# RaphaelHaddad/Real-Time-Brain-Inspired-Video-Memory

Hardware: AMD Instinct MI355X
Metric: frame-embeddings/sec (+ kNN queries/sec, see knn) (higher is better)
Workload: dtype f16; 1 GPU; BASELINE configs[1]: ViT-B/16-224 encoder fp16, chunks of 16 frames, cosine top-10 over a 100000-row x 768 fp16 memory shard per GPU; chunk_size=16, memory_rows_per_gpu=100000, top_k=10, parallelism=single GPU

## Files before the change

include/vidmem.h:

```cpp
#ifndef VIDMEM_H
#define VIDMEM_H

#include <stddef.h>
#include <stdint.h>

#ifdef __cplusplus
extern "C" {
#endif

typedef struct vm_ctx vm_ctx;
typedef struct vm_encoder vm_encoder;
typedef struct vm_memory vm_memory;

enum vm_status {
    VM_OK = 0,
    VM_ERR_INVALID = -1,
    VM_ERR_HIP = -2,
    VM_ERR_NOMEM = -3,
    VM_ERR_UNSUPPORTED = -4,
    VM_ERR_NO_DEVICE = -5
};
enum vm_dtype { VM_F16 = 0, VM_BF16 = 1, VM_F32 = 2  };
enum vm_act { VM_ACT_GELU = 0, VM_ACT_QUICK_GELU = 1 };
enum vm_layout { VM_LAYOUT_CHW = 0, VM_LAYOUT_PATCHES = 1 };
enum vm_score_mode { VM_SCORE_RAW = 0, VM_SCORE_UNIT_INTERVAL = 1 };
enum vm_topk_flag { VM_FLAG_CERTIFIED = 0, VM_FLAG_GAP = 1, VM_FLAG_OVERFLOW = 3 };

int vm_init(int device, vm_ctx **out);
void vm_destroy(vm_ctx *ctx);
const char *vm_last_error(vm_ctx *ctx);
int vm_abi_version(void);

int vm_preprocess(vm_ctx *ctx, const uint8_t *frames_hwc_bgr, int B, int H, int W, const float mean_host[3],
                  const float std_host[3], int out_S, int dtype, int layout, int patch, int k_pad, void *out,
                  void *stream);

typedef struct vm_encoder_desc {
    int image;
    int patch;
    int hidden;
    int layers;
    int heads;
    int mlp;
    int act;
    int pre_ln;
    int patch_bias;
    int proj_dim;
    int dtype;
    float ln_eps;
} vm_encoder_desc;

int vm_encoder_create(vm_ctx *ctx, const vm_encoder_desc *desc, const void *const *weights_host, int n_weights,
                      vm_encoder **out);
void vm_encoder_destroy(vm_encoder *enc);
enum vm_encoder_option { VM_ENC_OPT_SCHEDULE = 0, VM_ENC_OPT_MICRO_BATCH = 1, VM_ENC_OPT_LAST_LAYER = 2 };
enum vm_encoder_schedule { VM_SCHED_AUTO = 0, VM_SCHED_ONE_STREAM = 1, VM_SCHED_TWO_STREAMS = 2 };
int vm_encoder_set_option(vm_encoder *enc, int option, int value);
int vm_encoder_get_option(const vm_encoder *enc, int option);
int vm_encoder_tokens(const vm_encoder *enc);
int vm_encoder_patch_k(const vm_encoder *enc);
int vm_encoder_out_dim(const vm_encoder *enc);
size_t vm_encode_workspace_bytes(const vm_encoder *enc, int B);
int vm_encode_micro_batch(const vm_encoder *enc, int B);
int vm_encode(vm_encoder *enc, const void *patches, int B, void *out_emb, int l2_normalise, void *workspace,
              size_t workspace_bytes, void *stream);

typedef struct vm_text_encoder vm_text_encoder;
typedef struct vm_text_encoder_desc {
    int vocab;
    int context;
    int hidden;
    int layers;
    int heads;
    int mlp;
    int act;
    int proj_dim;
    int eot_id;
    int dtype;
    float ln_eps;
} vm_text_encoder_desc;
int vm_text_encoder_create(vm_ctx *ctx, const vm_text_encoder_desc *desc, const void *const *weights_host,
                           int n_weights, vm_text_encoder **out);
void vm_text_encoder_destroy(vm_text_encoder *enc);
int vm_text_encoder_out_dim(const vm_text_encoder *enc);
size_t vm_text_encode_workspace_bytes(const vm_text_encoder *enc, int B, int T);
int vm_text_encode(vm_text_encoder *enc, const int32_t *token_ids, int B, int T, void *out_emb, int l2_normalise,
                   int32_t *out_flags, void *workspace, size_t workspace_bytes, void *stream);

// ... 85 lines not shown
```

real-time-brain-inspired-video-memory_amd/_lib.py:

```python
from __future__ import annotations

import ctypes as C
import os
from typing import Optional

_HERE = os.path.dirname(os.path.abspath(__file__))
LIB_PATH = os.path.join(_HERE, "libvidmem.so")
DEV_LIB_PATH = os.path.join(_HERE, "libvidmem_dev.so")

VM_OK = 0
VM_ERR_INVALID, VM_ERR_HIP, VM_ERR_NOMEM, VM_ERR_UNSUPPORTED, VM_ERR_NO_DEVICE = -1, -2, -3, -4, -5
VM_F16, VM_BF16, VM_F32 = 0, 1, 2
VM_ACT_GELU, VM_ACT_QUICK_GELU = 0, 1
VM_LAYOUT_CHW, VM_LAYOUT_PATCHES = 0, 1
VM_SCORE_RAW, VM_SCORE_UNIT_INTERVAL = 0, 1
VM_FLAG_CERTIFIED, VM_FLAG_GAP, VM_FLAG_OVERFLOW = 0, 1, 3
VM_ENC_OPT_SCHEDULE, VM_ENC_OPT_MICRO_BATCH, VM_ENC_OPT_LAST_LAYER = 0, 1, 2
VM_SCHED_AUTO, VM_SCHED_ONE_STREAM, VM_SCHED_TWO_STREAMS = 0, 1, 2
SCHEDULES = {"auto": VM_SCHED_AUTO, "one_stream": VM_SCHED_ONE_STREAM, "two_streams": VM_SCHED_TWO_STREAMS}
DTYPES = {"f16": VM_F16, "bf16": VM_BF16}

SYMBOLS = [
    "vm_init", "vm_destroy", "vm_last_error", "vm_abi_version", "vm_preprocess",
    "vm_encoder_create", "vm_encoder_destroy", "vm_encoder_set_option", "vm_encoder_get_option",
    "vm_encoder_tokens", "vm_encoder_patch_k", "vm_encoder_out_dim",
    "vm_encode_workspace_bytes", "vm_encode_micro_batch", "vm_encode",
    "vm_memory_create", "vm_memory_destroy", "vm_memory_append", "vm_memory_size", "vm_memory_capacity",
    "vm_memory_dim", "vm_memory_reset", "vm_memory_sync", "vm_memory_rows",
    "vm_memory_create_grouped", "vm_memory_append_grouped", "vm_memory_group_keys",
    "vm_topk_grouped_workspace_bytes", "vm_topk_cosine_grouped", "vm_topk_cosine_grouped_exact",
    "vm_memory_create_tagged", "vm_memory_append_tagged", "vm_memory_tags",
    "vm_novelty_workspace_bytes", "vm_memory_append_novel",
    "vm_topk_scoped_workspace_bytes", "vm_topk_cosine_scoped", "vm_topk_cosine_scoped_exact",
    "vm_topk_workspace_bytes", "vm_topk_cosine", "vm_topk_redo_workspace_bytes", "vm_topk_redo_flagged",
    "vm_topk_exact_workspace_bytes", "vm_topk_cosine_exact",
    "vm_cosine_exact", "vm_topk_select", "vm_topk_merge", "vm_profile_enable", "vm_profile_read", "vm_profile_mask", "vm_probe_mfma",
    "vm_text_encoder_create", "vm_text_encoder_destroy", "vm_text_encoder_out_dim", "vm_text_encode_workspace_bytes",
    "vm_text_encode",
]
PROF_CATS = ["preprocess", "gemm_patch", "gemm_qkv", "gemm_act", "gemm_resid", "attention", "layernorm", "pool",
             "append", "topk_scan", "topk_finalize", "topk_exact", "topk_merge", "gemm_cls"]


class VidmemError(RuntimeError):
    def __init__(self, code: int, message: str):
        super().__init__(f"libvidmem error {code}: {message}")
        self.code = code


class EncoderDesc(C.Structure):
# ... 149 lines not shown
```

real-time-brain-inspired-video-memory_amd/csrc/encoder.hip:

```cpp
#include "vm_internal.h"
#include "vm_kernels.h"

#include <type_traits>

namespace {

__device__ __forceinline__ float wave_sum(float v) {
    auto dpp_add = [](float x, auto ctrl, auto row_mask) {
        const int y = __builtin_amdgcn_update_dpp(0, __builtin_bit_cast(int, x), decltype(ctrl)::value,
                                                  decltype(row_mask)::value, 0xf, false);
        return x + __builtin_bit_cast(float, y);
    };
    using std::integral_constant;
    v = dpp_add(v, integral_constant<int, 0xB1>{}, integral_constant<int, 0xf>{});
    v = dpp_add(v, integral_constant<int, 0x4E>{}, integral_constant<int, 0xf>{});
    v = dpp_add(v, integral_constant<int, 0x141>{}, integral_constant<int, 0xf>{});
    v = dpp_add(v, integral_constant<int, 0x140>{}, integral_constant<int, 0xf>{});
    v = dpp_add(v, integral_constant<int, 0x142>{}, integral_constant<int, 0xa>{});
    v = dpp_add(v, integral_constant<int, 0x143>{}, integral_constant<int, 0xc>{});
    return __builtin_bit_cast(float, __builtin_amdgcn_readlane(__builtin_bit_cast(int, v), 63));
}

typedef float f32x4_v __attribute__((ext_vector_type(4)));
typedef unsigned u32x2_v __attribute__((ext_vector_type(2)));
// ... 90 lines not shown
                v[r][i].w += e[r][i].w;
            }
        }
        if (write_x > 1 ? row % write_x == 0 : write_x) {
            float4 *xr = reinterpret_cast<float4 *>(x32 + (size_t)row * rstride * H);
#pragma unroll
            for (int i = 0; i < VPL; ++i) st_f4<NT>(xr + lane + 64 * i, v[r][i]);
        }
        float sum = 0.f;
#pragma unroll
        for (int i = 0; i < VPL; ++i) sum += (v[r][i].x + v[r][i].y) + (v[r][i].z + v[r][i].w);
        const float mean = wave_sum(sum) / (float)H;
        float sq = 0.f;
#pragma unroll
        for (int i = 0; i < VPL; ++i) {
            const float a = v[r][i].x - mean, b = v[r][i].y - mean, c = v[r][i].z - mean, e = v[r][i].w - mean;
            sq += (a * a + b * b) + (c * c + e * e);
        }
        const float rstd = rsqrtf(wave_sum(sq) / (float)H + eps);
#pragma unroll
        for (int i = 0; i < VPL; ++i) {
            uint16_t o[4] = {E::from_float((v[r][i].x - mean) * rstd * g4[i].x + b4[i].x),
                             E::from_float((v[r][i].y - mean) * rstd * g4[i].y + b4[i].y),
                             E::from_float((v[r][i].z - mean) * rstd * g4[i].z + b4[i].z),
                             E::from_float((v[r][i].w - mean) * rstd * g4[i].w + b4[i].w)};
            uint2 pk;
            __builtin_memcpy(&pk, o, 8);
            st_u2<NT>(reinterpret_cast<uint2 *>(out16 + (size_t)row * rstride * H) + lane + 64 * i, pk);
        }
    }
}

template <int DT, int VPL, bool NT>
__global__ void __launch_bounds__(256, 8) resid_layernorm_lowreg_kernel(float *__restrict__ x32,
                                                                        const uint16_t *__restrict__ delta16,
                                                                        const uint16_t *__restrict__ deltaB16,
                                                                        int write_x, const float *__restrict__ gamma,
                                                                        const float *__restrict__ beta, float eps,
                                                                        uint16_t *__restrict__ out16, int rows, int H,
                                                                        int rstride) {
    using E = vm_elem<DT>;
    const int lane = threadIdx.x & 63;
    const int row = blockIdx.x * 4 + (threadIdx.x >> 6);
    if (row >= rows) return;
    const size_t base = (size_t)row * rstride * H;
    float4 v[VPL];
    const float4 *xr = reinterpret_cast<const float4 *>(x32 + base);
#pragma unroll
    for (int i = 0; i < VPL; ++i) v[i] = ld_f4<NT>(xr + lane + 64 * i);
    if (delta16) {
        float4 d[VPL];
#pragma unroll
        for (int i = 0; i < VPL; ++i) d[i] = load4_16<VM_F16, NT>(delta16 + base + 4 * (lane + 64 * i));
#pragma unroll
        for (int i = 0; i < VPL; ++i) {
            v[i].x += d[i].x;
            v[i].y += d[i].y;
            v[i].z += d[i].z;
            v[i].w += d[i].w;
        }
    }
    if (deltaB16) {
        float4 d[VPL];
#pragma unroll
        for (int i = 0; i < VPL; ++i) d[i] = load4_16<VM_F16, NT>(deltaB16 + base + 4 * (lane + 64 * i));
#pragma unroll
        for (int i = 0; i < VPL; ++i) {
            v[i].x += d[i].x;
            v[i].y += d[i].y;
            v[i].z += d[i].z;
            v[i].w += d[i].w;
        }
    }
    if (write_x > 1 ? row % write_x == 0 : write_x) {
        float4 *xw = reinterpret_cast<float4 *>(x32 + base);
#pragma unroll
        for (int i = 0; i < VPL; ++i) st_f4<NT>(xw + lane + 64 * i, v[i]);
    }
    float sum = 0.f;
#pragma unroll
    for (int i = 0; i < VPL; ++i) sum += (v[i].x + v[i].y) + (v[i].z + v[i].w);
    const float mean = wave_sum(sum) / (float)H;
    float sq = 0.f;
#pragma unroll
    for (int i = 0; i < VPL; ++i) {
        const float a = v[i].x - mean, b = v[i].y - mean, c = v[i].z - mean, e = v[i].w - mean;
        sq += (a * a + b * b) + (c * c + e * e);
    }
    const float rstd = rsqrtf(wave_sum(sq) / (float)H + eps);
#pragma unroll
    for (int i = 0; i < VPL; ++i) {
        const float4 g4 = reinterpret_cast<const float4 *>(gamma)[lane + 64 * i];
        const float4 b4 = reinterpret_cast<const float4 *>(beta)[lane + 64 * i];
        uint16_t o[4] = {E::from_float((v[i].x - mean) * rstd * g4.x + b4.x),
                         E::from_float((v[i].y - mean) * rstd * g4.y + b4.y),
                         E::from_float((v[i].z - mean) * rstd * g4.z + b4.z),
                         E::from_float((v[i].w - mean) * rstd * g4.w + b4.w)};
        uint2 pk;
        __builtin_memcpy(&pk, o, 8);
        st_u2<NT>(reinterpret_cast<uint2 *>(out16 + base) + lane + 64 * i, pk);
    }
}

template <int DT, int VPL>
__global__ void __launch_bounds__(256) embed_kernel(const uint16_t *__restrict__ patch16, const float *__restrict__ cls,
                                                    const float *__restrict__ pos, const float *__restrict__ pre_g,
                                                    const float *__restrict__ pre_b, float eps, int pre_ln,
                                                    float *__restrict__ x32, int rows, int T, int H) {
    const int lane = threadIdx.x & 63;
    const int row = blockIdx.x * 4 + (threadIdx.x >> 6);
    if (row >= rows) return;
    const int frame = row / T, tok = row - frame * T;
    float4 v[VPL];
#pragma unroll
    for (int i = 0; i < VPL; ++i) {
        const int c = lane + 64 * i;
        const float4 p4 = reinterpret_cast<const float4 *>(pos + (size_t)tok * H)[c];
        float4 e4;
        if (tok == 0)
            e4 = reinterpret_cast<const float4 *>(cls)[c];
        else
            e4 = load4_16<VM_F16>(patch16 + ((size_t)frame * (T - 1) + tok - 1) * H + 4 * c);
        v[i] = make_float4(e4.x + p4.x, e4.y + p4.y, e4.z + p4.z, e4.w + p4.w);
    }
    if (pre_ln) {
        float sum = 0.f;
#pragma unroll
        for (int i = 0; i < VPL; ++i) sum += (v[i].x + v[i].y) + (v[i].z + v[i].w);
        const float mean = wave_sum(sum) / (float)H;
        float sq = 0.f;
#pragma unroll
        for (int i = 0; i < VPL; ++i) {
            const float a = v[i].x - mean, b = v[i].y - mean, c = v[i].z - mean, d = v[i].w - mean;
            sq += (a * a + b * b) + (c * c + d * d);
// ... 101 lines not shown
        const int tt = t0 + lane;
        const int v = tt < T ? ids[(size_t)b * T + tt] : 0;
        const unsigned long long hit = __ballot(tt < T && v == eot_id);
        if (hit && first == T) first = t0 + __ffsll((long long)hit) - 1;
        clamped |= __any(tt < T && (v < 0 || v >= vocab)) != 0;
    }
    if (lane == 0) {
        pool_row[b] = first < T ? first : 0;
        if (flags) flags[b] = (clamped ? 1 : 0) | (first < T ? 0 : 2);
    }
}

}

#define VM_VPL_SWITCH(H, CALL)                                                                     \
    switch ((H) / 256) {                                                                           \
        case 1: CALL(1); break;                                                                    \
        case 2: CALL(2); break;                                                                    \
        case 3: CALL(3); break;                                                                    \
        case 4: CALL(4); break;                                                                    \
        default: return vm_fail(ctx, VM_ERR_UNSUPPORTED, "row width %d (need 256..1024, %%256)", H); \
    }

int vm_resid_layernorm(vm_ctx *ctx, int dtype, float *x32, const uint16_t *delta16, const uint16_t *deltaB16,
                       int write_x, const float *gamma, const float *beta, float eps, uint16_t *out16, int rows, int H,
                       hipStream_t st, int rstride, int lowreg) {
    constexpr int RPW = 2;
    const int blocks = (rows + 4 * RPW - 1) / (4 * RPW);
    if (H % 256 != 0) return vm_fail(ctx, VM_ERR_UNSUPPORTED, "row width %d", H);
    vm_prof_scope prof(ctx, VM_PROF_LAYERNORM, st);
    static const int lowreg_env = (int)VM_DEV_ENV("LN_LOWREG", 1);
    if (lowreg != 0 && lowreg_env != 0) {
        const int blk = (rows + 3) / 4;
#define RLNL(V)                                                                                                          \
    if (dtype == VM_F16)                                                                                                 \
        resid_layernorm_lowreg_kernel<VM_F16, V, true><<<blk, 256, 0, st>>>(x32, delta16, deltaB16, write_x, gamma, beta, eps, out16, rows, H, rstride); \
    else                                                                                                                 \
        resid_layernorm_lowreg_kernel<VM_BF16, V, true><<<blk, 256, 0, st>>>(x32, delta16, deltaB16, write_x, gamma, beta, eps, out16, rows, H, rstride)
        VM_VPL_SWITCH(H, RLNL)
#undef RLNL
        VM_LAUNCH_CHECK(ctx);
        return VM_OK;
    }
    static const int nt_env = (int)VM_DEV_ENV("LN_NT", 1);
    const bool nt = nt_env && (size_t)rows * H * 4 > ((size_t)64 << 20);
#define RLN16(V) resid_layernorm_kernel<VM_F16, V, RPW, false><<<blocks, 256, 0, st>>>(x32, delta16, deltaB16, write_x, gamma, beta, eps, out16, rows, H, rstride)
#define RLNB16(V) resid_layernorm_kernel<VM_BF16, V, RPW, false><<<blocks, 256, 0, st>>>(x32, delta16, deltaB16, write_x, gamma, beta, eps, out16, rows, H, rstride)
#define RLN16N(V) resid_layernorm_kernel<VM_F16, V, RPW, true><<<blocks, 256, 0, st>>>(x32, delta16, deltaB16, write_x, gamma, beta, eps, out16, rows, H, rstride)
#define RLNB16N(V) resid_layernorm_kernel<VM_BF16, V, RPW, true><<<blocks, 256, 0, st>>>(x32, delta16, deltaB16, write_x, gamma, beta, eps, out16, rows, H, rstride)
    if (dtype == VM_F16) {
        if (nt) { VM_VPL_SWITCH(H, RLN16N) } else { VM_VPL_SWITCH(H, RLN16) }
    } else {
        if (nt) { VM_VPL_SWITCH(H, RLNB16N) } else { VM_VPL_SWITCH(H, RLNB16) }
    }
#undef RLN16
#undef RLNB16
#undef RLN16N
#undef RLNB16N
    VM_LAUNCH_CHECK(ctx);
    return VM_OK;
}

int vm_embed(vm_ctx *ctx, int dtype, const uint16_t *patch16, const float *cls, const float *pos, const float *pre_g,
             const float *pre_b, float eps, int pre_ln, float *x32, int B, int T, int H, hipStream_t st) {
    const int rows = B * T, blocks = (rows + 3) / 4;
    if (H % 256 != 0) return vm_fail(ctx, VM_ERR_UNSUPPORTED, "row width %d", H);
// ... 35 lines not shown
    const int rows = B * T, blocks = (rows + 3) / 4;
    if (H % 256 != 0) return vm_fail(ctx, VM_ERR_UNSUPPORTED, "row width %d", H);
    vm_prof_scope prof(ctx, VM_PROF_LAYERNORM, st);
#define TEMB(V) text_embed_kernel<V><<<blocks, 256, 0, st>>>(ids, tok, pos, vocab, eot_id, x32, pool_row, flags, rows, T, H)
    VM_VPL_SWITCH(H, TEMB)
#undef TEMB
    VM_LAUNCH_CHECK(ctx);
    return VM_OK;
}

struct LayerW {
    float *ln1_g, *ln1_b, *qkv_b, *proj_b, *ln2_g, *ln2_b, *fc1_b, *fc2_b;
    uint16_t *qkv_w, *proj_w, *fc1_w, *fc2_w;
};
static void layer_sizes(size_t H, size_t M, size_t lsz[12]) {
    const size_t v[12] = {H * 4, H * 4, 3 * H * H * 2, 3 * H * 4, H * H * 2, H * 4,
                          H * 4, H * 4, M * H * 2,     M * 4,     H * M * 2, H * 4};
    for (int i = 0; i < 12; ++i) lsz[i] = v[i];
}
static void bind_layer(LayerW &w, char *b, const size_t o[12]) {
    w.ln1_g = (float *)(b + o[0]);
    w.ln1_b = (float *)(b + o[1]);
    w.qkv_w = (uint16_t *)(b + o[2]);
    w.qkv_b = (float *)(b + o[3]);
    w.proj_w = (uint16_t *)(b + o[4]);
    w.proj_b = (float *)(b + o[5]);
    w.ln2_g = (float *)(b + o[6]);
    w.ln2_b = (float *)(b + o[7]);
    w.fc1_w = (uint16_t *)(b + o[8]);
    w.fc1_b = (float *)(b + o[9]);
    w.fc2_w = (uint16_t *)(b + o[10]);
    w.fc2_b = (float *)(b + o[11]);
}
struct vm_encoder {
    vm_ctx *ctx;
    vm_encoder_desc d;
    int tokens, patches, patch_k, out_dim;
    char *blob;
    uint16_t *patch_w, *proj_w;
    float *patch_b, *cls, *pos, *pre_g, *pre_b, *ln_g, *ln_b;
    LayerW *layers;
    int micro_batch;
    int cls_last;
    int schedule;
    hipStream_t side[2];
    hipEvent_t ev_fork, ev_join[2], ev_phase;
};

static int round_up(int x, int a) { return (x + a - 1) / a * a; }

extern "C" int vm_encoder_create(vm_ctx *ctx, const vm_encoder_desc *desc, const void *const *wp, int n_weights,
                                 vm_encoder **out) {
    if (!ctx || !desc || !wp || !out) return VM_ERR_INVALID;
    const vm_encoder_desc &d = *desc;
    if (d.hidden % 256 != 0 || d.hidden > 1024 || d.heads * 64 != d.hidden)
        return vm_fail(ctx, VM_ERR_UNSUPPORTED, "hidden=%d heads=%d: need hidden %% 256 == 0, <= 1024, head dim 64",
                       d.hidden, d.heads);
    if (d.mlp % 128 != 0 || d.image % d.patch != 0 || d.layers <= 0 || d.image % 8 != 0)
        return vm_fail(ctx, VM_ERR_UNSUPPORTED, "bad mlp/image/patch/layers");
    if (d.dtype != VM_F16 && d.dtype != VM_BF16) return vm_fail(ctx, VM_ERR_INVALID, "bad dtype");
    if (d.proj_dim < 0 || d.proj_dim % 8 != 0) return vm_fail(ctx, VM_ERR_UNSUPPORTED, "proj_dim %d", d.proj_dim);
    if (n_weights != 9 + 12 * d.layers)
        return vm_fail(ctx, VM_ERR_INVALID, "expected %d weight pointers, got %d", 9 + 12 * d.layers, n_weights);
    VM_HIP(ctx, hipSetDevice(ctx->device));
    vm_encoder *e = new vm_encoder();
    memset(e, 0, sizeof(*e));
    e->ctx = ctx;
    e->d = d;
    const int g = d.image / d.patch;
    e->patches = g * g;
    e->tokens = e->patches + 1;
    e->patch_k = round_up(3 * d.patch * d.patch, 64);
    e->out_dim = d.proj_dim ? d.proj_dim : d.hidden;
    if (e->tokens > 592) {
        const int tokens = e->tokens;
        delete e;
        return vm_fail(ctx, VM_ERR_UNSUPPORTED, "%d tokens per frame > 592", tokens);
    }
    e->micro_batch = 0;
    e->cls_last = 3;
    e->schedule = VM_SCHED_AUTO;
    {
        hipError_t he = hipSuccess;
        for (int i = 0; i < 2 && he == hipSuccess; ++i) {
            he = hipStreamCreateWithFlags(&e->side[i], hipStreamNonBlocking);
            if (he == hipSuccess) he = hipEventCreateWithFlags(&e->ev_join[i], hipEventDisableTiming);
        }
        if (he == hipSuccess) he = hipEventCreateWithFlags(&e->ev_fork, hipEventDisableTiming);
        if (he == hipSuccess) he = hipEventCreateWithFlags(&e->ev_phase, hipEventDisableTiming);
        if (he != hipSuccess) {
            vm_encoder_destroy(e);
            return vm_fail(ctx, VM_ERR_HIP, "encoder streams: %s", hipGetErrorString(he));
        }
    }
    const size_t H = d.hidden, M = d.mlp;
    auto a256 = [](size_t b) { return vm_align_up(b, 256); };
    size_t total = 0;
    auto take = [&](size_t bytes) {
        size_t off = total;
        total += a256(bytes);
        return off;
    };
    const size_t o_patch_w = take(H * e->patch_k * 2), o_patch_b = take(H * 4), o_cls = take(H * 4),
                 o_pos = take((size_t)e->tokens * H * 4), o_pre_g = take(H * 4), o_pre_b = take(H * 4),
                 o_ln_g = take(H * 4), o_ln_b = take(H * 4), o_proj = take((size_t)(d.proj_dim ? d.proj_dim : 0) * H * 2);
    struct LO {
        size_t o[12];
    };
    LO *lo = new LO[d.layers];
    size_t lsz[12];
    layer_sizes(H, M, lsz);
    for (int l = 0; l < d.layers; ++l)
        for (int i = 0; i < 12; ++i) lo[l].o[i] = take(lsz[i]);
    hipError_t er = hipMalloc((void **)&e->blob, total);
    if (er != hipSuccess) {
        delete[] lo;
        delete e;
        return vm_fail(ctx, VM_ERR_NOMEM, "encoder weights: hipMalloc(%zu) failed", total);
    }
    auto copy = [&](size_t off, const void *src, size_t bytes) -> hipError_t {
        if (bytes == 0) return hipSuccess;
        if (!src) return hipErrorInvalidValue;
// ... 5 lines not shown
    if (er == hipSuccess) er = copy(o_pos, wp[3], (size_t)e->tokens * H * 4);
    if (er == hipSuccess && d.pre_ln) er = copy(o_pre_g, wp[4], H * 4);
    if (er == hipSuccess && d.pre_ln) er = copy(o_pre_b, wp[5], H * 4);
    if (er == hipSuccess) er = copy(o_ln_g, wp[6], H * 4);
    if (er == hipSuccess) er = copy(o_ln_b, wp[7], H * 4);
    if (er == hipSuccess && d.proj_dim) er = copy(o_proj, wp[8], (size_t)d.proj_dim * H * 2);
    e->layers = new LayerW[d.layers];
    for (int l = 0; l < d.layers && er == hipSuccess; ++l) {
        for (int i = 0; i < 12 && er == hipSuccess; ++i) er = copy(lo[l].o[i], wp[9 + 12 * l + i], lsz[i]);
        bind_layer(e->layers[l], e->blob, lo[l].o);
    }
    delete[] lo;
    if (er != hipSuccess) {
        vm_encoder_destroy(e);
        return vm_fail(ctx, VM_ERR_HIP, "encoder weight copy failed: %s (null or short weight pointer?)",
                       hipGetErrorString(er));
    }
    char *b = e->blob;
    e->patch_w = (uint16_t *)(b + o_patch_w);
    e->patch_b = (float *)(b + o_patch_b);
    e->cls = (float *)(b + o_cls);
    e->pos = (float *)(b + o_pos);
    e->pre_g = (float *)(b + o_pre_g);
    e->pre_b = (float *)(b + o_pre_b);
    e->ln_g = (float *)(b + o_ln_g);
    e->ln_b = (float *)(b + o_ln_b);
    e->proj_w = d.proj_dim ? (uint16_t *)(b + o_proj) : nullptr;
    *out = e;
    return VM_OK;
}

extern "C" void vm_encoder_destroy(vm_encoder *e) {
    if (!e) return;
    for (int i = 0; i < 2; ++i) {
        if (e->side[i]) (void)hipStreamDestroy(e->side[i]);
        if (e->ev_join[i]) (void)hipEventDestroy(e->ev_join[i]);
    }
    if (e->ev_fork) (void)hipEventDestroy(e->ev_fork);
    if (e->ev_phase) (void)hipEventDestroy(e->ev_phase);
    if (e->blob) (void)hipFree(e->blob);
    delete[] e->layers;
    delete e;
}

extern "C" int vm_encoder_set_option(vm_encoder *e, int option, int value) {
    if (!e) return VM_ERR_INVALID;
    switch (option) {
        case VM_ENC_OPT_SCHEDULE:
            if (value != VM_SCHED_AUTO && value != VM_SCHED_ONE_STREAM && value != VM_SCHED_TWO_STREAMS)
                return vm_fail(e->ctx, VM_ERR_INVALID, "VM_ENC_OPT_SCHEDULE: %d", value);
            e->schedule = value;
            return VM_OK;
        case VM_ENC_OPT_MICRO_BATCH:
            if (value < 0) return vm_fail(e->ctx, VM_ERR_INVALID, "VM_ENC_OPT_MICRO_BATCH: %d", value);
            e->micro_batch = value;
            return VM_OK;
        case VM_ENC_OPT_LAST_LAYER:
            if (value != 0 && value != 1 && value != 3)
                return vm_fail(e->ctx, VM_ERR_INVALID, "VM_ENC_OPT_LAST_LAYER: %d (0, 1 or 3)", value);
            e->cls_last = value;
            return VM_OK;
        default:
            return vm_fail(e->ctx, VM_ERR_INVALID, "unknown encoder option %d", option);
    }
}
extern "C" int vm_encoder_get_option(const vm_encoder *e, int option) {
    if (!e) return VM_ERR_INVALID;
    switch (option) {
        case VM_ENC_OPT_SCHEDULE: return e->schedule;
        case VM_ENC_OPT_MICRO_BATCH: return e->micro_batch;
        case VM_ENC_OPT_LAST_LAYER: return e->cls_last;
        default: return VM_ERR_INVALID;
    }
}

extern "C" int vm_encoder_tokens(const vm_encoder *e) { return e ? e->tokens : 0; }
extern "C" int vm_encoder_patch_k(const vm_encoder *e) { return e ? e->patch_k : 0; }
extern "C" int vm_encoder_out_dim(const vm_encoder *e) { return e ? e->out_dim : 0; }

static int micro_batch_of(const vm_encoder *e, int B) {
    int mb = e->micro_batch;
    if (mb <= 0) {
        const int col_tiles = e->d.hidden / 256;
        const int row_tiles = 8 * (e->ctx->num_cus / col_tiles);
        mb = row_tiles * 256 / e->tokens;
        if (mb < 1) mb = 1;
        if (e->tokens > 208) {
            const int items = mb * e->d.heads, cus = e->ctx->num_cus;
            const int full = items / cus * cus;
            if (full > 0 && full % e->d.heads == 0 && (items - full) * 32 < items) mb = full / e->d.heads;
        }
    }
    return B < mb ? B : mb;
}

struct Ws {
    float *x32;
    uint16_t *a16, *d16, *e16, *qkv16, *mlp16;
    size_t bytes;
};
static Ws carve_rows(size_t rows, size_t H, size_t M, void *base) {
    Ws w;
    size_t off = 0;
    auto take = [&](size_t bytes) {
// ... 63 lines not shown
                              causal)) != VM_OK)
            return r;
        if (last_cls) {
            const int TH = T * H;
            return gemm16(ws.a16, TH, w.proj_w, w.proj_b, ws.d16, nb, H, H, EPI_DELTA16, VM_PROF_GEMM_CLS, TH);
        }
        return gemm16(ws.a16, H, w.proj_w, w.proj_b, ws.d16, rows, H, H, EPI_DELTA16, VM_PROF_GEMM_RESID);
    }
    int ln2(Pass &p, int l) const {
        const LayerW &w = lw[l];
        const bool last_cls = l == layers - 1 && cls_only();
        return vm_resid_layernorm(ctx, dt, p.ws.x32, p.ws.d16, nullptr, 0, w.ln2_g, w.ln2_b, eps, p.ws.a16,
                                  last_cls ? p.nb : p.rows, H, st, last_cls ? T : 1, dual && !last_cls ? 1 : 0);
    }
    int mlp_block(Pass &p, int l) const {
        const LayerW &w = lw[l];
        const Ws &ws = p.ws;
        const bool last_cls = l == layers - 1 && cls_only();
        int r;
        if (last_cls) {
            const int TH = T * H;
            if ((r = gemm16(ws.a16, TH, w.fc1_w, w.fc1_b, ws.mlp16, p.nb, mlp, H, act_epi, VM_PROF_GEMM_CLS)) != VM_OK) return r;
            r = gemm16(ws.mlp16, mlp, w.fc2_w, w.fc2_b, ws.e16, p.nb, H, mlp, EPI_DELTA16, VM_PROF_GEMM_CLS, TH);
        } else {
            if ((r = gemm16(ws.a16, H, w.fc1_w, w.fc1_b, ws.mlp16, p.rows, mlp, H, act_epi, VM_PROF_GEMM_ACT)) != VM_OK) return r;
            r = gemm16(ws.mlp16, mlp, w.fc2_w, w.fc2_b, ws.e16, p.rows, H, mlp, EPI_DELTA16, VM_PROF_GEMM_RESID);
        }
        p.pend_proj = ws.d16;
        p.pend_fc2 = ws.e16;
        return r;
    }
};

extern "C" size_t vm_encode_workspace_bytes(const vm_encoder *e, int B) {
    if (!e || B <= 0) return 0;
    const int mb = micro_batch_of(e, B);
    const size_t one = carve(e, mb, nullptr).bytes;
    return (e->schedule != VM_SCHED_ONE_STREAM && B > mb) ? 2 * one : one;
}

extern "C" int vm_encode_micro_batch(const vm_encoder *e, int B) { return e && B > 0 ? micro_batch_of(e, B) : 0; }

extern "C" int vm_encode(vm_encoder *e, const void *patches, int B, void *out_emb, int l2_normalise,
                         void *workspace, size_t workspace_bytes, void *stream) {
    if (!e) return VM_ERR_INVALID;
    vm_ctx *ctx = e->ctx;
    if (!patches || !out_emb || B <= 0) return vm_fail(ctx, VM_ERR_INVALID, "vm_encode: bad arguments");
    const int mb = micro_batch_of(e, B);
    const Ws ws0 = carve(e, mb, workspace);
    if (!workspace || workspace_bytes < ws0.bytes)
        return vm_fail(ctx, VM_ERR_NOMEM, "vm_encode: workspace %zu < %zu", workspace_bytes, ws0.bytes);
    if (((uintptr_t)workspace & 255) || ((uintptr_t)patches & 15) || ((uintptr_t)out_emb & 15))
        return vm_fail(ctx, VM_ERR_INVALID, "vm_encode: workspace must be 256-byte, tensors 16-byte aligned");
    hipStream_t st = (hipStream_t)stream;
    const vm_encoder_desc &d = e->d;
    const int H = d.hidden, T = e->tokens, P = e->patches, dt = d.dtype;
    const int act_epi = d.act == VM_ACT_QUICK_GELU ? EPI_QGELU16 : EPI_GELU16;
    const int cls_env = e->cls_last;

    const bool timing = ctx->prof_ev != nullptr;
    const bool dual = B > mb && workspace_bytes >= 2 * ws0.bytes &&
                      (e->schedule == VM_SCHED_TWO_STREAMS || (e->schedule == VM_SCHED_AUTO && !timing));
    const Ws ws1 = dual ? carve(e, mb, (char *)workspace + ws0.bytes) : ws0;
    hipStream_t st0 = st;
    int rc = VM_OK;
    if (dual) {
        VM_HIP(ctx, hipEventRecord(e->ev_fork, st0));
        for (int i = 0; i < 2; ++i) VM_HIP(ctx, hipStreamWaitEvent(e->side[i], e->ev_fork, 0));
    }
    Tower tw;
    tw.ctx = ctx; tw.dt = dt; tw.H = H; tw.heads = d.heads; tw.mlp = d.mlp; tw.act_epi = act_epi; tw.layers = d.layers;
    tw.T = T; tw.eps = d.ln_eps; tw.lw = e->layers; tw.cls_env = cls_env; tw.dual = dual; tw.causal = 0; tw.st = st;
    auto embed = [&](Pass &p) -> int {
        int r = tw.gemm16((const uint16_t *)patches + (size_t)p.b0 * P * e->patch_k, e->patch_k, e->patch_w, e->patch_b,
                          p.ws.d16, p.nb * P, H, e->patch_k, EPI_DELTA16, VM_PROF_GEMM_PATCH);
        if (r != VM_OK) return r;
        p.pend_proj = p.pend_fc2 = nullptr;
        return vm_embed(ctx, dt, p.ws.d16, e->cls, e->pos, e->pre_g, e->pre_b, d.ln_eps, d.pre_ln, p.ws.x32, p.nb, T, H, st);
    };
    auto pool = [&](Pass &p) -> int {
        uint16_t *dst = (uint16_t *)out_emb + (size_t)p.b0 * e->out_dim;
        return vm_pool(ctx, dt, p.ws.x32, p.pend_proj, p.pend_fc2, e->ln_g, e->ln_b, d.ln_eps, e->proj_w, d.proj_dim,
                       l2_normalise, dst, p.nb, T, H, st);
    };
#define VM_TRY(x) do { if ((rc = (x)) != VM_OK) return rc; } while (0)
    auto run_passes = [&]() -> int {
        int pass = 0;
        for (int b0 = 0; b0 < B; ++pass) {
            Pass A;
            A.b0 = b0;
            A.nb = B - b0 < mb ? B - b0 : mb;
            A.rows = A.nb * T;
            A.ws = dual && (pass & 1) ? ws1 : ws0;
            st = tw.st = dual ? e->side[pass & 1] : st0;
            static const int phase_env = (int)VM_DEV_ENV("ENC_PHASE", 0);
            const bool mark = dual && phase_env > 0 && pass == 0;
            if (dual && phase_env > 0 && pass == 1) (void)hipStreamWaitEvent(st, e->ev_phase, 0);
            VM_TRY(embed(A));
            for (int l = 0; l < d.layers; ++l) {
                VM_TRY(tw.ln1(A, l));
                if (mark && l == 0 && phase_env == 1) (void)hipEventRecord(e->ev_phase, st);
                VM_TRY(tw.attn_block(A, l));
                if (mark && l == 0 && phase_env == 2) (void)hipEventRecord(e->ev_phase, st);
                VM_TRY(tw.ln2(A, l));
                if (mark && l == 0 && phase_env == 3) (void)hipEventRecord(e->ev_phase, st);
                VM_TRY(tw.mlp_block(A, l));
                if (mark && l == 0 && phase_env == 4) (void)hipEventRecord(e->ev_phase, st);
                if (mark && l == 1 && phase_env == 5) (void)hipEventRecord(e->ev_phase, st);
            }
            VM_TRY(pool(A));
            b0 += A.nb;
        }
        return VM_OK;
    };
#undef VM_TRY
    rc = run_passes();
    if (dual) {
        for (int i = 0; i < 2; ++i) {
            hipError_t he = hipEventRecord(e->ev_join[i], e->side[i]);
            if (he == hipSuccess) he = hipStreamWaitEvent(st0, e->ev_join[i], 0);
            if (he != hipSuccess && rc == VM_OK)
                rc = vm_fail(ctx, VM_ERR_HIP, "vm_encode: joining the internal streams failed: %s", hipGetErrorString(he));
        }
    }
    return rc;
}

struct vm_text_encoder {
    vm_ctx *ctx;
    vm_text_encoder_desc d;
    int out_dim;
    char *blob;
    float *tok, *pos, *ln_g, *ln_b;
    uint16_t *proj_w;
    LayerW *layers;
};

extern "C" int vm_text_encoder_create(vm_ctx *ctx, const vm_text_encoder_desc *desc, const void *const *wp, int n_weights,
                                      vm_text_encoder **out) {
    if (!ctx || !desc || !wp || !out) return VM_ERR_INVALID;
    const vm_text_encoder_desc &d = *desc;
    if (d.hidden % 256 != 0 || d.hidden > 1024 || d.heads * 64 != d.hidden)
        return vm_fail(ctx, VM_ERR_UNSUPPORTED, "text hidden=%d heads=%d: need hidden %% 256 == 0, <= 1024, head dim 64",
                       d.hidden, d.heads);
    if (d.mlp % 128 != 0 || d.layers <= 0 || d.vocab <= 0 || d.context < 1 || d.context > 80)
        return vm_fail(ctx, VM_ERR_UNSUPPORTED, "text tower: bad mlp/layers/vocab or context %d (1..80)", d.context);
    if (d.dtype != VM_F16 && d.dtype != VM_BF16) return vm_fail(ctx, VM_ERR_INVALID, "bad dtype");
    if (d.act != VM_ACT_GELU && d.act != VM_ACT_QUICK_GELU) return vm_fail(ctx, VM_ERR_INVALID, "bad act %d", d.act);
    if (d.proj_dim < 0 || d.proj_dim % 8 != 0) return vm_fail(ctx, VM_ERR_UNSUPPORTED, "proj_dim %d", d.proj_dim);
    if (n_weights != 5 + 12 * d.layers)
        return vm_fail(ctx, VM_ERR_INVALID, "expected %d weight pointers, got %d", 5 + 12 * d.layers, n_weights);
// ... 115 lines not shown
```

real-time-brain-inspired-video-memory_amd/encoder.py:

```python
from __future__ import annotations

import ctypes as C
from typing import Dict, List, Optional, Sequence

import numpy as np
import torch

from . import _lib
from .memory import _torch_dtype


def _weight_order(spec: Dict) -> List[str]:
    names = ["patch_w", "patch_b", "cls", "pos", "pre_ln_g", "pre_ln_b", "ln_g", "ln_b", "proj_w"]
    for l in range(spec["layers"]):
        names += [f"l{l}.{n}" for n in ("ln1_g", "ln1_b", "qkv_w", "qkv_b", "proj_w", "proj_b", "ln2_g", "ln2_b",
                                        "fc1_w", "fc1_b", "fc2_w", "fc2_b")]
    return names


_MATRICES = ("patch_w", "proj_w", "qkv_w", "fc1_w", "fc2_w")


class FrameEncoder:

    def __init__(self, spec: Dict, weights: Dict[str, np.ndarray], dtype: str = "f16", device: int = 0,
                 schedule: str = "auto", micro_batch: int = 0, last_layer: int = 3):
        self.spec = dict(spec)
        self.ctx = _lib.Context.get(device)
        self.L = self.ctx.L
        self.device = torch.device("cuda", device)
        self.dtype_name = dtype
        self.dtype = _torch_dtype(dtype)
        self.patch_k = (3 * spec["patch"] ** 2 + 63) // 64 * 64
        desc = _lib.EncoderDesc(
            image=spec["image"], patch=spec["patch"], hidden=spec["hidden"], layers=spec["layers"],
            heads=spec["heads"], mlp=spec["mlp"],
            act=_lib.VM_ACT_QUICK_GELU if spec["act"] == "quick_gelu" else _lib.VM_ACT_GELU,
            pre_ln=int(bool(spec["pre_ln"])), patch_bias=int(bool(spec["patch_bias"])),
            proj_dim=int(spec.get("proj_dim", 0)), dtype=_lib.DTYPES[dtype], ln_eps=float(spec["ln_eps"]))
        staged = []
        ptrs = []
        for name in _weight_order(spec):
            arr = weights.get(name)
            if arr is None:
                ptrs.append(None)
                continue
            t = torch.as_tensor(np.asarray(arr), dtype=torch.float32)
            if name.split(".")[-1] in _MATRICES:
                if name == "patch_w" and t.shape[1] < self.patch_k:
                    t = torch.nn.functional.pad(t, (0, self.patch_k - t.shape[1]))
                t = t.to(self.dtype)
            t = t.to(self.device).contiguous()
            staged.append(t)
            ptrs.append(t.data_ptr())
        arr_t = (C.c_void_p * len(ptrs))(*[C.c_void_p(p) if p else C.c_void_p(0) for p in ptrs])
        h = C.c_void_p()
        torch.cuda.synchronize(self.device)
        self.ctx.check(self.L.vm_encoder_create(self.ctx.handle, C.byref(desc), arr_t, len(ptrs), C.byref(h)))
        torch.cuda.synchronize(self.device)
        del staged
        self.handle = h
        self.tokens = int(self.L.vm_encoder_tokens(h))
        self.out_dim = int(self.L.vm_encoder_out_dim(h))
        assert int(self.L.vm_encoder_patch_k(h)) == self.patch_k
        self.set_schedule(schedule)
        if micro_batch:
            self.set_option(_lib.VM_ENC_OPT_MICRO_BATCH, int(micro_batch))
        if last_layer != 3:
            self.set_option(_lib.VM_ENC_OPT_LAST_LAYER, int(last_layer))
        self._ws = None
        self._mean = (C.c_float * 3)(*spec["mean"])
        self._std = (C.c_float * 3)(*spec["std"])

    def set_option(self, option: int, value: int) -> None:
        self.ctx.check(self.L.vm_encoder_set_option(self.handle, int(option), int(value)))

    def set_schedule(self, schedule: str) -> None:
        if schedule not in _lib.SCHEDULES:
            raise ValueError(f"schedule must be one of {sorted(_lib.SCHEDULES)}")
        self.set_option(_lib.VM_ENC_OPT_SCHEDULE, _lib.SCHEDULES[schedule])

    @property
    def schedule(self) -> str:
        v = int(self.L.vm_encoder_get_option(self.handle, _lib.VM_ENC_OPT_SCHEDULE))
        return {n: k for k, n in _lib.SCHEDULES.items()}[v]

    def close(self):
        if getattr(self, "handle", None):
            self.L.vm_encoder_destroy(self.handle)
            self.handle = None

    def __del__(self):
        try:
            self.close()
        except Exception:
            pass

    def preprocess(self, frames_u8: torch.Tensor, layout: str = "patches") -> torch.Tensor:
        if frames_u8.dtype != torch.uint8 or frames_u8.dim() != 4 or frames_u8.shape[-1] != 3:
            raise ValueError("frames must be uint8 [B,H,W,3] (BGR, as cv2.VideoCapture.read returns them)")
        f = frames_u8.to(self.device).contiguous()
        B, Hh, Ww, _ = f.shape
        S, p = self.spec["image"], self.spec["patch"]
        if layout == "patches":
            out = torch.empty((B, (S // p) ** 2, self.patch_k), dtype=self.dtype, device=self.device)
            lay = _lib.VM_LAYOUT_PATCHES
        else:
            out = torch.empty((B, 3, S, S), dtype=self.dtype, device=self.device)
            lay = _lib.VM_LAYOUT_CHW
        self.ctx.check(self.L.vm_preprocess(
            self.ctx.handle, C.c_void_p(f.data_ptr()), B, Hh, Ww, self._mean, self._std, S,
            _lib.DTYPES[self.dtype_name], lay, p, self.patch_k, C.c_void_p(out.data_ptr()), _lib.current_stream_ptr()))
        f.record_stream(torch.cuda.current_stream())
        return out

    def patches_from_pixels(self, pixels_chw: torch.Tensor) -> torch.Tensor:
        B, Cc, S, _ = pixels_chw.shape
        p = self.spec["patch"]
# ... 57 lines not shown
```

Measured before the change: 26810 frame-embeddings/s.

## Split encoder micro-batches into concurrent stream chains and specialize LayerNorm for H=768

Restructures the encoder schedule so each micro-batch workspace can be split into several frame slices, each a chain on its own stream (up to three side streams). By default stages are issued interleaved across chains, so small kernels from different slices can overlap and fill the GPU. Slice sizes are rounded to multiples of frames that fill the CUs for one round. It also adds a dedicated residual+LayerNorm kernel for hidden=768 that uses asm barriers to keep register pressure low. This costs extra stream and event traffic, and slicing shrinks each GEMM, which may lower per-kernel efficiency.

```diff
diff --git a/include/vidmem.h b/include/vidmem.h
--- a/include/vidmem.h
+++ b/include/vidmem.h
@@ -53,7 +53,8 @@
 int vm_encoder_create(vm_ctx *ctx, const vm_encoder_desc *desc, const void *const *weights_host, int n_weights,
                       vm_encoder **out);
 void vm_encoder_destroy(vm_encoder *enc);
-enum vm_encoder_option { VM_ENC_OPT_SCHEDULE = 0, VM_ENC_OPT_MICRO_BATCH = 1, VM_ENC_OPT_LAST_LAYER = 2 };
+enum vm_encoder_option { VM_ENC_OPT_SCHEDULE = 0, VM_ENC_OPT_MICRO_BATCH = 1, VM_ENC_OPT_LAST_LAYER = 2,
+                         VM_ENC_OPT_SLICES = 3, VM_ENC_OPT_STREAMS_USED = 4 };
 enum vm_encoder_schedule { VM_SCHED_AUTO = 0, VM_SCHED_ONE_STREAM = 1, VM_SCHED_TWO_STREAMS = 2 };
 int vm_encoder_set_option(vm_encoder *enc, int option, int value);
 int vm_encoder_get_option(const vm_encoder *enc, int option);
diff --git a/real-time-brain-inspired-video-memory_amd/_lib.py b/real-time-brain-inspired-video-memory_amd/_lib.py
--- a/real-time-brain-inspired-video-memory_amd/_lib.py
+++ b/real-time-brain-inspired-video-memory_amd/_lib.py
@@ -15,7 +15,7 @@
 VM_LAYOUT_CHW, VM_LAYOUT_PATCHES = 0, 1
 VM_SCORE_RAW, VM_SCORE_UNIT_INTERVAL = 0, 1
 VM_FLAG_CERTIFIED, VM_FLAG_GAP, VM_FLAG_OVERFLOW = 0, 1, 3
-VM_ENC_OPT_SCHEDULE, VM_ENC_OPT_MICRO_BATCH, VM_ENC_OPT_LAST_LAYER = 0, 1, 2
+VM_ENC_OPT_SCHEDULE, VM_ENC_OPT_MICRO_BATCH, VM_ENC_OPT_LAST_LAYER, VM_ENC_OPT_SLICES, VM_ENC_OPT_STREAMS_USED = 0, 1, 2, 3, 4
 VM_SCHED_AUTO, VM_SCHED_ONE_STREAM, VM_SCHED_TWO_STREAMS = 0, 1, 2
 SCHEDULES = {"auto": VM_SCHED_AUTO, "one_stream": VM_SCHED_ONE_STREAM, "two_streams": VM_SCHED_TWO_STREAMS}
 DTYPES = {"f16": VM_F16, "bf16": VM_BF16}
diff --git a/real-time-brain-inspired-video-memory_amd/csrc/encoder.hip b/real-time-brain-inspired-video-memory_amd/csrc/encoder.hip
--- a/real-time-brain-inspired-video-memory_amd/csrc/encoder.hip
+++ b/real-time-brain-inspired-video-memory_amd/csrc/encoder.hip
@@ -146,13 +146,10 @@
 }
 
 template <int DT, int VPL, bool NT>
-__global__ void __launch_bounds__(256, 8) resid_layernorm_lowreg_kernel(float *__restrict__ x32,
-                                                                        const uint16_t *__restrict__ delta16,
-                                                                        const uint16_t *__restrict__ deltaB16,
-                                                                        int write_x, const float *__restrict__ gamma,
-                                                                        const float *__restrict__ beta, float eps,
-                                                                        uint16_t *__restrict__ out16, int rows, int H,
-                                                                        int rstride) {
+__device__ __forceinline__ void resid_layernorm_row(float *__restrict__ x32, const uint16_t *__restrict__ delta16,
+                                                    const uint16_t *__restrict__ deltaB16, int write_x,
+                                                    const float *__restrict__ gamma, const float *__restrict__ beta,
+                                                    float eps, uint16_t *__restrict__ out16, int rows, int H, int rstride) {
     using E = vm_elem<DT>;
     const int lane = threadIdx.x & 63;
     const int row = blockIdx.x * 4 + (threadIdx.x >> 6);
@@ -214,6 +211,84 @@
         __builtin_memcpy(&pk, o, 8);
         st_u2<NT>(reinterpret_cast<uint2 *>(out16 + base) + lane + 64 * i, pk);
     }
+}
+
+template <int DT, int VPL, bool NT>
+__global__ void __launch_bounds__(256, 8) resid_layernorm_lowreg_kernel(float *__restrict__ x32,
+                                                                        const uint16_t *__restrict__ delta16,
+                                                                        const uint16_t *__restrict__ deltaB16,
+                                                                        int write_x, const float *__restrict__ gamma,
+                                                                        const float *__restrict__ beta, float eps,
+                                                                        uint16_t *__restrict__ out16, int rows, int H,
+                                                                        int rstride) {
+    resid_layernorm_row<DT, VPL, NT>(x32, delta16, deltaB16, write_x, gamma, beta, eps, out16, rows, H, rstride);
+}
+
+template <int DT, bool NT>
+__global__ void __launch_bounds__(256)
+resid_layernorm_lowreg32_kernel(float *__restrict__ x32, const uint16_t *__restrict__ delta16,
+                                const uint16_t *__restrict__ deltaB16, int write_x, const float *__restrict__ gamma,
+                                const float *__restrict__ beta, float eps, uint16_t *__restrict__ out16, int rows, int H,
+                                int rstride) {
+    using E = vm_elem<DT>;
+    constexpr int VPL = 3;
+    const int lane = threadIdx.x & 63;
+    const int row = blockIdx.x * 4 + (threadIdx.x >> 6);
+    if (row >= rows) return;
+    const bool fold_x = write_x > 1 ? row % write_x == 0 : write_x != 0;
+    size_t el = (size_t)row * rstride * H + 4 * lane;
+#define VM_FORGET(x) asm volatile("" : "+v"(x))
+    float4 v[VPL];
+#pragma unroll
+    for (int i = 0; i < VPL; ++i) v[i] = ld_f4<NT>(reinterpret_cast<const float4 *>(x32 + el) + 64 * i);
+    auto fold = [&](const uint16_t *__restrict__ d16) {
+        VM_FORGET(el);
+        float4 d[VPL];
+#pragma unroll
+        for (int i = 0; i < VPL; ++i) d[i] = load4_16<VM_F16, NT>(d16 + el + 256 * i);
+#pragma unroll
+        for (int i = 0; i < VPL; ++i) {
+            v[i].x += d[i].x;
+            v[i].y += d[i].y;
+            v[i].z += d[i].z;
+            v[i].w += d[i].w;
+        }
+    };
+    if (delta16) fold(delta16);
+    if (deltaB16) fold(deltaB16);
+    if (fold_x) {
+        VM_FORGET(el);
+#pragma unroll
+        for (int i = 0; i < VPL; ++i) st_f4<NT>(reinterpret_cast<float4 *>(x32 + el) + 64 * i, v[i]);
+    }
+    float sum = 0.f;
+#pragma unroll
+    for (int i = 0; i < VPL; ++i) sum += (v[i].x + v[i].y) + (v[i].z + v[i].w);
+    const float mean = wave_sum(sum) / (float)H;
+    float sq = 0.f;
+#pragma unroll
+    for (int i = 0; i < VPL; ++i) {
+        const float a = v[i].x - mean, b = v[i].y - mean, c = v[i].z - mean, e = v[i].w - mean;
+        sq += (a * a + b * b) + (c * c + e * e);
+    }
+    const float rstd = rsqrtf(wave_sum(sq) / (float)H + eps);
+    int col = lane;
+    asm volatile("" : "+v"(col) : "v"(rstd));
+    VM_FORGET(el);
+#pragma unroll
+    for (int i = 0; i < VPL; ++i) {
+        const float4 g4 = reinterpret_cast<const float4 *>(gamma)[col + 64 * i];
+        const float4 b4 = reinterpret_cast<const float4 *>(beta)[col + 64 * i];
+        uint16_t o[4] = {E::from_float((v[i].x - mean) * rstd * g4.x + b4.x),
+                         E::from_float((v[i].y - mean) * rstd * g4.y + b4.y),
+                         E::from_float((v[i].z - mean) * rstd * g4.z + b4.z),
+                         E::from_float((v[i].w - mean) * rstd * g4.w + b4.w)};
+        uint2 pk;
+        __builtin_memcpy(&pk, o, 8);
+        asm volatile("" : "+v"(col) : "v"(pk.x), "v"(pk.y));
+        st_u2<NT>(reinterpret_cast<uint2 *>(out16 + el) + 64 * i, pk);
+    }
+#undef VM_FORGET
 }
 
 template <int DT, int VPL>
@@ -381,6 +456,15 @@
     static const int lowreg_env = (int)VM_DEV_ENV("LN_LOWREG", 1);
     if (lowreg != 0 && lowreg_env != 0) {
         const int blk = (rows + 3) / 4;
+        static const int ln32_env = (int)VM_DEV_ENV("LN_32", 1);
+        if (H == 768 && ln32_env != 0) {
+            if (dtype == VM_F16)
+                resid_layernorm_lowreg32_kernel<VM_F16, true><<<blk, 256, 0, st>>>(x32, delta16, deltaB16, write_x, gamma, beta, eps, out16, rows, H, rstride);
+            else
+                resid_layernorm_lowreg32_kernel<VM_BF16, true><<<blk, 256, 0, st>>>(x32, delta16, deltaB16, write_x, gamma, beta, eps, out16, rows, H, rstride);
+            VM_LAUNCH_CHECK(ctx);
+            return VM_OK;
+        }
 #define RLNL(V)                                                                                                          \
     if (dtype == VM_F16)                                                                                                 \
         resid_layernorm_lowreg_kernel<VM_F16, V, true><<<blk, 256, 0, st>>>(x32, delta16, deltaB16, write_x, gamma, beta, eps, out16, rows, H, rstride); \
@@ -482,6 +566,7 @@
     w.fc2_w = (uint16_t *)(b + o[10]);
     w.fc2_b = (float *)(b + o[11]);
 }
+enum { VM_ENC_SIDE_STREAMS = 3, VM_ENC_MAX_CHAINS = VM_ENC_SIDE_STREAMS + 1 };
 struct vm_encoder {
     vm_ctx *ctx;
     vm_encoder_desc d;
@@ -493,8 +578,10 @@
     int micro_batch;
     int cls_last;
     int schedule;
-    hipStream_t side[2];
-    hipEvent_t ev_fork, ev_join[2], ev_phase;
+    int slices;
+    int last_streams;
+    hipStream_t side[VM_ENC_SIDE_STREAMS];
+    hipEvent_t ev_fork, ev_join[VM_ENC_SIDE_STREAMS];
 };
 
 static int round_up(int x, int a) { return (x + a - 1) / a * a; }
@@ -530,14 +617,15 @@
     e->micro_batch = 0;
     e->cls_last = 3;
     e->schedule = VM_SCHED_AUTO;
+    e->slices = 0;
+    e->last_streams = 0;
     {
         hipError_t he = hipSuccess;
-        for (int i = 0; i < 2 && he == hipSuccess; ++i) {
+        for (int i = 0; i < VM_ENC_SIDE_STREAMS && he == hipSuccess; ++i) {
             he = hipStreamCreateWithFlags(&e->side[i], hipStreamNonBlocking);
             if (he == hipSuccess) he = hipEventCreateWithFlags(&e->ev_join[i], hipEventDisableTiming);
         }
         if (he == hipSuccess) he = hipEventCreateWithFlags(&e->ev_fork, hipEventDisableTiming);
-        if (he == hipSuccess) he = hipEventCreateWithFlags(&e->ev_phase, hipEventDisableTiming);
         if (he != hipSuccess) {
             vm_encoder_destroy(e);
             return vm_fail(ctx, VM_ERR_HIP, "encoder streams: %s", hipGetErrorString(he));
@@ -609,12 +697,11 @@
 
 extern "C" void vm_encoder_destroy(vm_encoder *e) {
     if (!e) return;
-    for (int i = 0; i < 2; ++i) {
+    for (int i = 0; i < VM_ENC_SIDE_STREAMS; ++i) {
         if (e->side[i]) (void)hipStreamDestroy(e->side[i]);
         if (e->ev_join[i]) (void)hipEventDestroy(e->ev_join[i]);
     }
     if (e->ev_fork) (void)hipEventDestroy(e->ev_fork);
-    if (e->ev_phase) (void)hipEventDestroy(e->ev_phase);
     if (e->blob) (void)hipFree(e->blob);
     delete[] e->layers;
     delete e;
@@ -637,6 +724,13 @@
                 return vm_fail(e->ctx, VM_ERR_INVALID, "VM_ENC_OPT_LAST_LAYER: %d (0, 1 or 3)", value);
             e->cls_last = value;
             return VM_OK;
+        case VM_ENC_OPT_SLICES:
+            if (value < 0 || value > VM_ENC_MAX_CHAINS)
+                return vm_fail(e->ctx, VM_ERR_INVALID, "VM_ENC_OPT_SLICES: %d (0 = auto, 1..%d)", value, VM_ENC_MAX_CHAINS);
+            e->slices = value;
+            return VM_OK;
+        case VM_ENC_OPT_STREAMS_USED:
+            return vm_fail(e->ctx, VM_ERR_INVALID, "VM_ENC_OPT_STREAMS_USED is read-only");
         default:
             return vm_fail(e->ctx, VM_ERR_INVALID, "unknown encoder option %d", option);
     }
@@ -647,6 +741,8 @@
         case VM_ENC_OPT_SCHEDULE: return e->schedule;
         case VM_ENC_OPT_MICRO_BATCH: return e->micro_batch;
         case VM_ENC_OPT_LAST_LAYER: return e->cls_last;
+        case VM_ENC_OPT_SLICES: return e->slices;
+        case VM_ENC_OPT_STREAMS_USED: return e->last_streams;
         default: return VM_ERR_INVALID;
     }
 }
@@ -776,6 +872,25 @@
     }
 };
 
+static int round_frames(const vm_encoder *e) {
+    const int row_tiles = e->ctx->num_cus / (e->d.hidden / 256);
+    const int f = row_tiles * 256 / e->tokens;
+    return f < 1 ? 1 : f;
+}
+static int split_frames(const vm_encoder *e, int frames, int parts, int *sizes) {
+    const int rf = round_frames(e), rounds = frames / rf;
+    if (rounds >= parts && parts > 1) {
+        for (int k = 0; k < parts; ++k) sizes[k] = (rounds / parts + (k < rounds % parts ? 1 : 0)) * rf;
+        sizes[parts - 1] += frames - rounds * rf;
+    } else {
+        for (int k = 0; k < parts; ++k) sizes[k] = frames / parts + (k < frames % parts ? 1 : 0);
+    }
+    return parts;
+}
+static int default_slices(const vm_encoder *e, int mb, int workspaces) {
+    return workspaces == 1 && mb >= 2 * round_frames(e) ? 2 : 1;
+}
+
 extern "C" size_t vm_encode_workspace_bytes(const vm_encoder *e, int B) {
     if (!e || B <= 0) return 0;
     const int mb = micro_batch_of(e, B);
@@ -803,14 +918,43 @@
     const int cls_env = e->cls_last;
 
     const bool timing = ctx->prof_ev != nullptr;
-    const bool dual = B > mb && workspace_bytes >= 2 * ws0.bytes &&
-                      (e->schedule == VM_SCHED_TWO_STREAMS || (e->schedule == VM_SCHED_AUTO && !timing));
-    const Ws ws1 = dual ? carve(e, mb, (char *)workspace + ws0.bytes) : ws0;
+    const bool multi = e->schedule == VM_SCHED_TWO_STREAMS || (e->schedule == VM_SCHED_AUTO && !timing);
+    const int W = multi && B > mb && workspace_bytes >= 2 * ws0.bytes ? 2 : 1;
+    int S = 1;
+    if (e->schedule == VM_SCHED_AUTO && !timing) {
+        S = e->slices ? e->slices : default_slices(e, mb, W);
+        if (S > VM_ENC_MAX_CHAINS / W) S = VM_ENC_MAX_CHAINS / W;
+    }
+    static const int chains_env = (int)VM_DEV_ENV("ENC_CHAINS", 0);
+    const bool flat = chains_env >= 1 && chains_env <= VM_ENC_MAX_CHAINS && e->schedule == VM_SCHED_AUTO && !timing;
+    struct Chain {
+        int f0, cap;
+        Ws ws;
+        hipStream_t st;
+    } chain[VM_ENC_MAX_CHAINS];
+    int K = 0;
+    {
+        int sizes[VM_ENC_MAX_CHAINS];
+        if (flat) {
+            K = split_frames(e, W * mb, chains_env, sizes);
+        } else {
+            for (int w = 0; w < W; ++w) K += split_frames(e, mb, S, sizes + K);
+        }
+        for (int k = 0, f0 = 0; k < K; f0 += sizes[k], ++k) {
+            chain[k].f0 = f0;
+            chain[k].cap = sizes[k];
+            chain[k].ws = carve(e, sizes[k], (char *)workspace + carve(e, f0, nullptr).bytes);
+        }
+    }
+    const bool dual = K > 1;
+    const int n_side = !dual ? 0 : K < VM_ENC_SIDE_STREAMS ? K : VM_ENC_SIDE_STREAMS;
     hipStream_t st0 = st;
+    for (int k = 0; k < K; ++k) chain[k].st = k < n_side ? e->side[k] : st0;
+    e->last_streams = dual ? K : 1;
     int rc = VM_OK;
     if (dual) {
         VM_HIP(ctx, hipEventRecord(e->ev_fork, st0));
-        for (int i = 0; i < 2; ++i) VM_HIP(ctx, hipStreamWaitEvent(e->side[i], e->ev_fork, 0));
+        for (int i = 0; i < n_side; ++i) VM_HIP(ctx, hipStreamWaitEvent(e->side[i], e->ev_fork, 0));
     }
     Tower tw;
     tw.ctx = ctx; tw.dt = dt; tw.H = H; tw.heads = d.heads; tw.mlp = d.mlp; tw.act_epi = act_epi; tw.layers = d.layers;
@@ -827,40 +971,53 @@
         return vm_pool(ctx, dt, p.ws.x32, p.pend_proj, p.pend_fc2, e->ln_g, e->ln_b, d.ln_eps, e->proj_w, d.proj_dim,
                        l2_normalise, dst, p.nb, T, H, st);
     };
-#define VM_TRY(x) do { if ((rc = (x)) != VM_OK) return rc; } while (0)
-    auto run_passes = [&]() -> int {
-        int pass = 0;
-        for (int b0 = 0; b0 < B; ++pass) {
-            Pass A;
-            A.b0 = b0;
-            A.nb = B - b0 < mb ? B - b0 : mb;
-            A.rows = A.nb * T;
-            A.ws = dual && (pass & 1) ? ws1 : ws0;
-            st = tw.st = dual ? e->side[pass & 1] : st0;
-            static const int phase_env = (int)VM_DEV_ENV("ENC_PHASE", 0);
-            const bool mark = dual && phase_env > 0 && pass == 0;
-            if (dual && phase_env > 0 && pass == 1) (void)hipStreamWaitEvent(st, e->ev_phase, 0);
-            VM_TRY(embed(A));
-            for (int l = 0; l < d.layers; ++l) {
-                VM_TRY(tw.ln1(A, l));
-                if (mark && l == 0 && phase_env == 1) (void)hipEventRecord(e->ev_phase, st);
-                VM_TRY(tw.attn_block(A, l));
-                if (mark && l == 0 && phase_env == 2) (void)hipEventRecord(e->ev_phase, st);
-                VM_TRY(tw.ln2(A, l));
-                if (mark && l == 0 && phase_env == 3) (void)hipEventRecord(e->ev_phase, st);
-                VM_TRY(tw.mlp_block(A, l));
-                if (mark && l == 0 && phase_env == 4) (void)hipEventRecord(e->ev_phase, st);
-                if (mark && l == 1 && phase_env == 5) (void)hipEventRecord(e->ev_phase, st);
+    const int n_stages = 2 + 4 * d.layers;
+    auto stage = [&](Pass &p, hipStream_t on, int i) -> int {
+        st = tw.st = on;
+        if (i == 0) return embed(p);
+        if (i == n_stages - 1) return pool(p);
+        const int l = (i - 1) / 4;
+        switch ((i - 1) % 4) {
+            case 0: return tw.ln1(p, l);
+            case 1: return tw.attn_block(p, l);
+            case 2: return tw.ln2(p, l);
+            default: return tw.mlp_block(p, l);
+        }
+    };
+    static const int order_env = (int)VM_DEV_ENV("ENC_ORDER", 0);
+    const bool by_stage = order_env ? order_env == 2 : e->schedule != VM_SCHED_TWO_STREAMS;
+    auto run_chains = [&]() -> int {
+        const int hold = W * mb;
+        for (int base = 0; base < B; base += hold) {
+            Pass A[VM_ENC_MAX_CHAINS];
+            hipStream_t on[VM_ENC_MAX_CHAINS];
+            int n = 0;
+            for (int k = 0; k < K && base + chain[k].f0 < B; ++k) {
+                if (chain[k].cap == 0) continue;
+                Pass &p = A[n];
+                p.b0 = base + chain[k].f0;
+                p.nb = B - p.b0 < chain[k].cap ? B - p.b0 : chain[k].cap;
+                p.rows = p.nb * T;
+                p.ws = chain[k].ws;
+                p.pend_proj = p.pend_fc2 = nullptr;
+                on[n++] = chain[k].st;
             }
-            VM_TRY(pool(A));
-            b0 += A.nb;
+            int r;
+            if (by_stage) {
+                for (int i = 0; i < n_stages; ++i)
+                    for (int c = 0; c < n; ++c)
+                        if ((r = stage(A[c], on[c], i)) != VM_OK) return r;
+            } else {
+                for (int c = 0; c < n; ++c)
+                    for (int i = 0; i < n_stages; ++i)
+                        if ((r = stage(A[c], on[c], i)) != VM_OK) return r;
+            }
         }
         return VM_OK;
     };
-#undef VM_TRY
-    rc = run_passes();
+    rc = run_chains();
     if (dual) {
-        for (int i = 0; i < 2; ++i) {
+        for (int i = 0; i < n_side; ++i) {
             hipError_t he = hipEventRecord(e->ev_join[i], e->side[i]);
             if (he == hipSuccess) he = hipStreamWaitEvent(st0, e->ev_join[i], 0);
             if (he != hipSuccess && rc == VM_OK)
diff --git a/real-time-brain-inspired-video-memory_amd/encoder.py b/real-time-brain-inspired-video-memory_amd/encoder.py
--- a/real-time-brain-inspired-video-memory_amd/encoder.py
+++ b/real-time-brain-inspired-video-memory_amd/encoder.py
@@ -24,7 +24,7 @@
 class FrameEncoder:
 
     def __init__(self, spec: Dict, weights: Dict[str, np.ndarray], dtype: str = "f16", device: int = 0,
-                 schedule: str = "auto", micro_batch: int = 0, last_layer: int = 3):
+                 schedule: str = "auto", micro_batch: int = 0, last_layer: int = 3, slices: int = 0):
         self.spec = dict(spec)
         self.ctx = _lib.Context.get(device)
         self.L = self.ctx.L
@@ -68,6 +68,8 @@
             self.set_option(_lib.VM_ENC_OPT_MICRO_BATCH, int(micro_batch))
         if last_layer != 3:
             self.set_option(_lib.VM_ENC_OPT_LAST_LAYER, int(last_layer))
+        if slices:
+            self.set_option(_lib.VM_ENC_OPT_SLICES, int(slices))
         self._ws = None
         self._mean = (C.c_float * 3)(*spec["mean"])
         self._std = (C.c_float * 3)(*spec["std"])
@@ -84,6 +86,10 @@
     def schedule(self) -> str:
         v = int(self.L.vm_encoder_get_option(self.handle, _lib.VM_ENC_OPT_SCHEDULE))
         return {n: k for k, n in _lib.SCHEDULES.items()}[v]
+
+    @property
+    def streams_used(self) -> int:
+        return int(self.L.vm_encoder_get_option(self.handle, _lib.VM_ENC_OPT_STREAMS_USED))
 
     def close(self):
         if getattr(self, "handle", None):
```

After: 26990 frame-embeddings/s, median of 6. Within noise of the previous version (+0.7%).
